# Rafae1130/qwen_inference_engine

Measured on AMD Instinct MI355X. Metric: decode tokens/s + prefill tok/s, Qwen2-7B bf16 batch=1, 1/2/4/8 MI355X, higher is better.
Workload: dtype bf16; 1 GPU; Qwen2-7B bf16 decode, batch=1, prompt=2048, gen=512; batch_per_gpu=1, batch=1, prompt=2048, gen=512, parallelism=single, graph=True, kv=contiguous

## Files before the change

### include/qie/qie_ops.h

```cpp
#ifndef QIE_OPS_H
#define QIE_OPS_H

#include "qie_types.h"

#ifdef __cplusplus
extern "C" {
#endif

#define QIE_ABI_VERSION 1

const char* qie_last_error(void);
int qie_abi_version(void);
int qie_device_count(int* count);

int qie_set_device(int device);
int qie_malloc(void** ptr, int64_t bytes);
int qie_free(void* ptr);
int qie_memcpy_h2d(void* dst, const void* src, int64_t bytes);
int qie_memcpy_d2h(void* dst, const void* src, int64_t bytes);
int qie_memset(void* ptr, int value, int64_t bytes);
int qie_synchronize(void);
int qie_stream_create(void** stream_out);
int qie_stream_synchronize(void* stream);
int qie_stream_destroy(void* stream);
// ... 23 lines not shown
    int64_t M, K, N;
    void* y;
    int64_t ldy;
    int32_t epilogue;
    int32_t numerics;
    const void* norm_w;
    float norm_eps;
    int32_t flags;
    uint64_t* argmax_keys;
    int64_t key_col0;
    const uint8_t* x_exps;
} qie_linear_args;

int qie_linear(const qie_linear_args* args, void* stream);

typedef struct qie_kv_cache {
    void* k;
    void* v;
    int64_t seq_stride;
    int32_t n_layers, n_kv_heads, head_dim, max_ctx;
    const int32_t* block_table;
    int32_t page_tokens;
    int32_t max_pages;
} qie_kv_cache;

int qie_qkv_post(const void* qkv, int64_t M, const int32_t* pos, int32_t rows_per_seq,
                 const void* q_norm, const void* k_norm, const float* rope_cos,
                 const float* rope_sin, int32_t n_heads, const qie_kv_cache* cache,
                 int32_t layer, float eps, int32_t numerics, void* q_out, void* stream);

int64_t qie_attention_workspace_bytes(int64_t M, int32_t n_heads, int32_t head_dim,
                                      int32_t max_ctx);
int qie_attention(const void* q, int64_t M, const int32_t* pos, int32_t rows_per_seq,
                  const qie_kv_cache* cache, int32_t layer, int32_t n_heads, void* out,
                  void* ws, void* stream);

int64_t qie_attention_extend_workspace_bytes(int64_t M, int32_t n_heads, int32_t head_dim,
                                             int32_t max_ctx);
int32_t qie_attention_extend_split_tokens(int64_t M, int32_t max_ctx);
int qie_attention_extend(const void* q, int64_t M, const int32_t* pos, int32_t rows_per_seq,
                         const qie_kv_cache* cache, int32_t layer, int32_t n_heads, void* out,
                         void* ws, void* stream);

#define QIE_NUMERICS_MASK 0xff
#define QIE_ATTN_PREROPED 0x100
int64_t qie_attention_decode_workspace_bytes(int64_t B, int32_t n_heads, int32_t n_kv_heads,
                                             int32_t head_dim, int32_t max_ctx);
int qie_attention_decode(const void* qkv, int64_t B, const int32_t* pos, const void* q_norm,
                         const void* k_norm, const float* rope_cos, const float* rope_sin,
                         int32_t n_heads, const qie_kv_cache* cache, int32_t layer, float eps,
                         int32_t numerics, void* out, void* ws, void* stream);

int qie_debug_tr16_probe(int32_t* out_dev);

int qie_qknorm(void* x, int64_t rows, int64_t row_stride, int32_t n_heads, int32_t head_dim,
               const void* w, float eps, int32_t numerics, void* stream);
int qie_rope(void* x, int64_t rows, int64_t row_stride, int32_t n_heads, int32_t head_dim,
             const int32_t* pos, int32_t pos0, const float* rope_cos, const float* rope_sin,
             int32_t numerics, void* stream);
int qie_kv_write(const void* k, const void* v, int64_t rows, int64_t ld, int32_t pos0,
                 const qie_kv_cache* cache, int32_t seq, int32_t layer, void* stream);

int qie_silu(void* x, int64_t n, void* stream);
int qie_mul(const void* a, const void* b, void* c, int64_t n, void* stream);
int qie_memcpy_d2d(void* dst, const void* src, int64_t bytes, void* stream);
int qie_silu_mul(const void* gate, const void* up, void* h, int64_t n, void* stream);
int qie_residual_add(void* x, const void* y, int64_t n, void* stream);
int qie_residual_add_f32(void* x, const float* sum, int64_t n, void* stream);

int64_t qie_sample_workspace_bytes(int64_t M, int64_t V);
int qie_sample(const void* logits, int64_t M, int64_t V, int64_t ld, const qie_sampling* s,
               const int32_t* step_dev, int32_t* out_ids, void* ws, void* stream);
int qie_keys_to_ids(const uint64_t* keys, int64_t M, int32_t* out_ids, void* stream);

uint32_t qie_tensor_id(const char* name);
int qie_synthetic_fill(void* dev, int64_t n, uint32_t tensor_id, uint64_t seed, float scale,
                       float offset, void* stream);
int qie_synthetic_fill_host(void* host, int64_t n, uint32_t tensor_id, uint64_t seed,
                            float scale, float offset);
#define QIE_LINEAR_FP8 1
#define QIE_LINEAR_TILE256 2
#define QIE_LINEAR_TILE128 4
#define QIE_LINEAR_STREAMK 8
int64_t qie_fp8_weight_bytes(int64_t rows, int64_t cols);
int qie_quantize_fp8(const void* w_bf16, int64_t rows, int64_t cols, void* out, void* stream);
int qie_quantize_fp8_host(const void* w_bf16, int64_t rows, int64_t cols, void* out);
int qie_dequantize_fp8(const void* w_fp8, int64_t rows, int64_t cols, void* out_bf16, void* stream);
#define QIE_LINEAR_FP8_T16 16
#define QIE_LINEAR_ACT_FP8 32
int qie_quantize_rows_fp8(const void* x, int64_t ldx, int64_t rows, int64_t cols, void* q, int64_t ldq,
                          void* exps, void* stream);
int qie_fp8_tile16(const void* w_fp8, int64_t rows, int64_t cols, void* out, void* stream);
int qie_debug_fp8_decode(float* out_dev);
int qie_debug_fp8_decode_bf16(uint16_t* out_dev);

int qie_synthetic_fill_slice(void* dev, int64_t rows, int64_t cols, int64_t full_cols, int64_t row0,
                             int64_t col0, uint32_t tensor_id, uint64_t seed, float scale, float offset,
                             void* stream);
int qie_scale_rows_pow2(void* w, int64_t rows, int64_t cols, int64_t row0, int64_t every, int32_t log2f,
                        void* stream);

#ifdef __cplusplus
}
#endif

#endif
```

### qwen_inference_engine_amd/_lib.py

```python
from __future__ import annotations

import ctypes as C
import os

_HERE = os.path.dirname(os.path.abspath(__file__))
LIB_PATH = os.environ.get("QIE_LIB") or os.path.join(_HERE, "lib", "libqie.so")

QIE_NUMERICS_REF = 0
QIE_NUMERICS_HF = 1
QIE_EPI_STORE = 0
QIE_EPI_RESIDUAL = 1
QIE_EPI_SWIGLU = 2
QIE_EPI_F32 = 3
QIE_LINEAR_FP8 = 1
QIE_LINEAR_TILE256 = 2
QIE_LINEAR_TILE128 = 4
QIE_LINEAR_STREAMK = 8
QIE_LINEAR_FP8_T16 = 16
QIE_LINEAR_ACT_FP8 = 32
QIE_ATTN_PREROPED = 0x100
QIE_COMM_ID_BYTES = 128
QIE_COMM_PEER_HANDLE_BYTES = 128


class ModelSpecC(C.Structure):
    _fields_ = [
        ("n_layers", C.c_int32), ("hidden", C.c_int32), ("n_heads", C.c_int32),
        ("n_kv_heads", C.c_int32), ("head_dim", C.c_int32), ("ffn", C.c_int32),
        ("vocab", C.c_int32), ("tie_embeddings", C.c_int32), ("qkv_bias", C.c_int32),
        ("qk_norm", C.c_int32), ("rms_eps", C.c_float), ("rope_theta", C.c_float),
        ("numerics", C.c_int32), ("reserved", C.c_int32 * 7),
    ]


class LayerWeightsC(C.Structure):
    _fields_ = [(n, C.c_void_p) for n in (
        "attn_norm", "wq", "wk", "wv", "bq", "bk", "bv", "q_norm", "k_norm", "wo",
        "ffn_norm", "w_gate", "w_up", "w_down")]


class ModelWeightsC(C.Structure):
    _fields_ = [("embed", C.c_void_p), ("final_norm", C.c_void_p), ("lm_head", C.c_void_p),
                ("n_layers", C.c_int32), ("layers", C.POINTER(LayerWeightsC))]


class SamplingC(C.Structure):
    _fields_ = [("top_k", C.c_int32), ("temperature", C.c_float), ("top_p", C.c_float),
                ("seed", C.c_uint64)]


class LinearArgsC(C.Structure):
    _fields_ = [
        ("x", C.c_void_p), ("ldx", C.c_int64), ("w", C.c_void_p * 3), ("bias", C.c_void_p * 3),
        ("seg_rows", C.c_int64 * 3), ("M", C.c_int64), ("K", C.c_int64), ("N", C.c_int64),
        ("y", C.c_void_p), ("ldy", C.c_int64), ("epilogue", C.c_int32), ("numerics", C.c_int32),
        ("norm_w", C.c_void_p), ("norm_eps", C.c_float), ("flags", C.c_int32),
        ("argmax_keys", C.c_void_p), ("key_col0", C.c_int64), ("x_exps", C.c_void_p),
    ]


class KvCacheC(C.Structure):
    _fields_ = [("k", C.c_void_p), ("v", C.c_void_p), ("seq_stride", C.c_int64),
                ("n_layers", C.c_int32), ("n_kv_heads", C.c_int32), ("head_dim", C.c_int32),
                ("max_ctx", C.c_int32), ("block_table", C.c_void_p), ("page_tokens", C.c_int32),
                ("max_pages", C.c_int32)]


class EngineOptsC(C.Structure):
    _fields_ = [("device", C.c_int32), ("max_ctx", C.c_int32), ("use_graph", C.c_int32),
                ("tp_rank", C.c_int32), ("tp_size", C.c_int32), ("tp_comm", C.c_void_p),
                ("weight_fp8", C.c_int32), ("comm_always", C.c_int32), ("prefill_fp8", C.c_int32),
                ("reserved", C.c_int32 * 5)]


_P = C.c_void_p
_I32, _I64, _U32, _U64, _F = C.c_int32, C.c_int64, C.c_uint32, C.c_uint64, C.c_float
_PI32 = C.POINTER(C.c_int32)
_PI64 = C.POINTER(C.c_int64)
_PF = C.POINTER(C.c_float)
_PD = C.POINTER(C.c_double)
_PCC = C.POINTER(C.c_char_p)
SIGNATURES = [
    ("qie_last_error", C.c_char_p, []),
    ("qie_abi_version", C.c_int, []),
    ("qie_device_count", C.c_int, [C.POINTER(C.c_int)]),
    ("qie_set_device", C.c_int, [C.c_int]),
    ("qie_malloc", C.c_int, [C.POINTER(_P), _I64]),
    ("qie_free", C.c_int, [_P]),
    ("qie_memcpy_h2d", C.c_int, [_P, _P, _I64]),
    ("qie_memcpy_d2h", C.c_int, [_P, _P, _I64]),
    ("qie_memset", C.c_int, [_P, C.c_int, _I64]),
    ("qie_synchronize", C.c_int, []),
    ("qie_stream_create", C.c_int, [C.POINTER(_P)]),
    ("qie_stream_synchronize", C.c_int, [_P]),
    ("qie_stream_destroy", C.c_int, [_P]),
    ("qie_rope_table_host", C.c_int, [_PF, _PF, _I32, _I32, _F, _I32]),
    ("qie_embedding", C.c_int, [_P, _P, _P, _I64, _I64, _P]),
    ("qie_rmsnorm", C.c_int, [_P, _P, _P, _I64, _I64, _F, _I32, _P]),
    ("qie_linear", C.c_int, [C.POINTER(LinearArgsC), _P]),
    ("qie_qkv_post", C.c_int, [_P, _I64, _P, _I32, _P, _P, _P, _P, _I32, C.POINTER(KvCacheC),
                               _I32, _F, _I32, _P, _P]),
    ("qie_attention_workspace_bytes", C.c_int64, [_I64, _I32, _I32, _I32]),
# ... 118 lines not shown
```

### qwen_inference_engine_amd/csrc/k_gemm.hip

```cpp
#include "qie_common.hpp"
#include "launch_util.hpp"
#include "../../include/qie/qie_ops.h"

#include <map>
#include <mutex>

namespace qie {

typedef __bf16 bf16x8 __attribute__((ext_vector_type(8)));
typedef float f32x4 __attribute__((ext_vector_type(4)));

struct GemmParams {
    const uint16_t* A;
    int64_t lda;
    const uint16_t* w0;
    const uint16_t* w1;
    const uint16_t* w2;
    const uint16_t* b0;
    const uint16_t* b1;
    const uint16_t* b2;
    int64_t n0, n01;
    int64_t M, K, N;
    int64_t wrows;
    uint16_t* C;
    int64_t ldc;
};

constexpr int BM = 128, BN = 128, BK = 64;

template <int EPI>
__device__ __forceinline__ const uint16_t* w_row(const GemmParams& p, int64_t nblk, int c, bool& valid, int eb,
                                                 int64_t& row, float& scale) {
    auto at = [&](const uint16_t* w, int64_t rows, int64_t r) {
        const uint8_t* b = reinterpret_cast<const uint8_t*>(w);
        scale = eb == 1 ? reinterpret_cast<const float*>(b + rows * p.K)[r] : 1.f;
        row = r;
        return reinterpret_cast<const uint16_t*>(b + r * p.K * eb);
    };
    if constexpr (EPI == QIE_EPI_SWIGLU) {
        const int64_t j = nblk * 64 + 32 * (c >> 6) + (c & 31);
        valid = j < p.N;
        const int64_t jj = valid ? j : p.N - 1;
        return ((c >> 5) & 1) ? at(p.w1, p.N, jj) : at(p.w0, p.N, jj);
    } else {
        const int64_t r = nblk * BN + c;
        valid = r < p.N;
        const int64_t rr = valid ? r : p.N - 1;
        if (rr < p.n0) return at(p.w0, p.n0, rr);
        if (rr < p.n01) return at(p.w1, p.n01 - p.n0, rr - p.n0);
        return at(p.w2, p.N - p.n01, rr - p.n01);
    }
}

__device__ __forceinline__ uint4 fp8x8_to_bf16(uint2 q, float sc) {
    float f[8];
    fp8x4_to_f32(q.x, f);
    fp8x4_to_f32(q.y, f + 4);
    return make_uint4(pack2(f[0] * sc, f[1] * sc), pack2(f[2] * sc, f[3] * sc), pack2(f[4] * sc, f[5] * sc),
                      pack2(f[6] * sc, f[7] * sc));
}

template <int EPI, int WT>
__global__ __launch_bounds__(256) void gemm_kernel(GemmParams p) {
#pragma clang fp contract(off)
    extern __shared__ __attribute__((aligned(16))) unsigned char smem[];
    uint16_t* As = reinterpret_cast<uint16_t*>(smem);
    uint16_t* Bs = reinterpret_cast<uint16_t*>(smem + 2 * BM * BK * 2);

    const int tid = threadIdx.x, lane = tid & 63, wave = tid >> 6;
    const int wr = wave >> 1, wc = wave & 1;
    const int64_t mblk = blockIdx.x, nblk = blockIdx.y;
    const int64_t m0 = mblk * BM;

    const uint16_t* a_src[4];
    const uint8_t* b_src[4];
    float b_sc[4];
    int lds_off[4];
    constexpr int EB = WT ? 1 : 2;
#pragma unroll
    for (int i = 0; i < 4; i++) {
        const int c = tid + 256 * i;
        const int row = c >> 3, ch = c & 7;
        int64_t ar = m0 + row;
        if (ar >= p.M) ar = p.M - 1;
// ... 225 lines not shown
        const uint16_t* Bs = As + TM * TK;
        bf16x8 af[8], bfr[NJ];
#pragma unroll
        for (int j = 0; j < NJ; j++) {
            const int row = wn * (BNT / 4) + j * 16 + fr;
            bfr[j] = *reinterpret_cast<const bf16x8*>(Bs + row * TK + ((g ^ big_swz(row)) * 8));
        }
#pragma unroll
        for (int i = 0; i < 8; i++) {
            const int row = wm * 128 + i * 16 + fr;
            af[i] = *reinterpret_cast<const bf16x8*>(As + row * TK + ((g ^ big_swz(row)) * 8));
        }
        __builtin_amdgcn_sched_barrier(0);
#pragma unroll
        for (int i = 0; i < 8; i++)
#pragma unroll
            for (int j = 0; j < NJ; j++)
                acc[i][j] = __builtin_amdgcn_mfma_f32_16x16x32_bf16(af[i], bfr[j], acc[i][j], 0, 0, 0);
    }

    if constexpr (EPI == QIE_EPI_SWIGLU) {
#pragma unroll
        for (int i = 0; i < 8; i++) {
#pragma unroll
            for (int jj = 0; jj < NJ / 2; jj++) {
                const int64_t col = nt * (BNT / 2) + (BNT / 8) * wn + 16 * jj + fr;
                if (col >= p.N) continue;
#pragma unroll
                for (int r = 0; r < 4; r++) {
                    const int64_t row = m0 + wm * 128 + i * 16 + g * 4 + r;
                    if (row >= p.M) continue;
                    const float gg = rbf(acc[i][jj][r]);
                    const float uu = rbf(acc[i][jj + NJ / 2][r]);
                    const float av = rbf(gg * (1.0f / (1.0f + expf(-gg))));
                    p.C[row * p.ldc + col] = f2bf(uu * av);
                }
            }
        }
    } else {
#pragma unroll
        for (int j = 0; j < NJ; j++) {
            const int64_t col = nt * BNT + wn * (BNT / 4) + j * 16 + fr;
            if (col >= p.N) continue;
            float bias = 0.f;
            if constexpr (EPI == QIE_EPI_STORE) {
                const uint16_t* b = col < p.n0 ? p.b0 : (col < p.n01 ? p.b1 : p.b2);
                if (b) bias = bf2f(b[col < p.n0 ? col : (col < p.n01 ? col - p.n0 : col - p.n01)]);
            }
#pragma unroll
            for (int i = 0; i < 8; i++) {
#pragma unroll
                for (int r = 0; r < 4; r++) {
                    const int64_t row = m0 + wm * 128 + i * 16 + g * 4 + r;
                    if (row >= p.M) continue;
                    if constexpr (EPI == QIE_EPI_F32) {
                        reinterpret_cast<float*>(p.C)[row * p.ldc + col] = acc[i][j][r];
                        continue;
                    }
                    uint16_t* dst = p.C + row * p.ldc + col;
                    if constexpr (EPI == QIE_EPI_RESIDUAL)
                        *dst = f2bf(bf2f(*dst) + rbf(acc[i][j][r]));
                    else
                        *dst = f2bf(acc[i][j][r] + bias);
                }
            }
        }
    }
}

typedef unsigned int u32x4_g8 __attribute__((ext_vector_type(4)));
namespace g8 {
constexpr int BM = 256, BN = 256, BK = 64;
constexpr int BUF = (BM + BN) * BK * 2;
}

__device__ __forceinline__ int g8_swz(int r) { return (r >> 1) & 7; }

struct G8Split {
    int splitk;
    float* slab;
    unsigned* cnt;
};

template <int EPI>
__global__ __launch_bounds__(512) void gemm8_kernel(GemmParams p, int n_mt, G8Split sk) {
#pragma clang fp contract(off)
    extern __shared__ __attribute__((aligned(16))) unsigned char smem[];
    const int tid = threadIdx.x, lane = tid & 63;
    const int wave = __builtin_amdgcn_readfirstlane(tid >> 6);
    const int wm = wave >> 2, wn = wave & 3;
    const int fr = lane & 15, g = lane >> 4;
    const int nwg = gridDim.x, orig = blockIdx.x;
    const int q8 = nwg >> 3, r8 = nwg & 7, xcd = orig & 7;
    const int wid = (xcd < r8 ? xcd * (q8 + 1) : r8 * (q8 + 1) + (xcd - r8) * q8) + (orig >> 3);
    const int tile = wid / sk.splitk, part = wid % sk.splitk;
    const int64_t mt = tile % n_mt, nt = tile / n_mt;
    const int64_t m0 = mt * g8::BM;

    const uint16_t* src[4][2];
    int dst_row[4][2];
#pragma unroll
    for (int u = 0; u < 4; u++)
#pragma unroll
        for (int i = 0; i < 2; i++) {
            const int b = 2 * wave + i;
            int row0;
            if (u == 0 || u == 3) row0 = (b < 8 ? 8 * b : 128 + 8 * (b - 8)) + (u == 3 ? 64 : 0);
            else row0 = 64 * (b >> 2) + 8 * (b & 3) + (u == 2 ? 32 : 0);
            dst_row[u][i] = row0;
            const int r = row0 + (lane >> 3);
            const int cs = (lane & 7) ^ g8_swz(r);
            if (u == 0 || u == 3) {
                int64_t ar = m0 + r;
                ar = ar < p.M ? ar : p.M - 1;
                src[u][i] = p.A + ar * p.lda + cs * 8;
            } else {
                src[u][i] = big_wrow<EPI, 256>(p, nt, r) + cs * 8;
            }
        }
    const int nk_all = (int)(p.K / g8::BK);
    const int kb = (int)((int64_t)part * nk_all / sk.splitk);
    const int nk = (int)((int64_t)(part + 1) * nk_all / sk.splitk) - kb;
    auto stage = [&](int u, int kt) {
        unsigned char* buf = smem + (kt & 1) * g8::BUF + ((u == 0 || u == 3) ? 0 : g8::BM * 128);
        const int64_t k0 = (int64_t)(kb + kt) * g8::BK;
#pragma unroll
        for (int i = 0; i < 2; i++) glds16(src[u][i] + k0, buf + dst_row[u][i] * 128);
    };

    f32x4 acc[8][4];
#pragma unroll
    for (int i = 0; i < 8; i++)
#pragma unroll
        for (int j = 0; j < 4; j++) acc[i][j] = f32x4{0.f, 0.f, 0.f, 0.f};
    bf16x8 fa[4][2], fb0[2][2], fb1[2][2];

    auto read_a = [&](const unsigned char* buf, int qa) {
#pragma unroll
        for (int i = 0; i < 4; i++)
#pragma unroll
            for (int s2 = 0; s2 < 2; s2++) {
                const int row = 128 * wm + 64 * qa + 16 * i + fr;
                fa[i][s2] = *reinterpret_cast<const bf16x8*>(buf + row * 128 + (((4 * s2 + g) ^ g8_swz(row)) * 16));
            }
    };
    auto read_b = [&](const unsigned char* buf, int qb, bf16x8 (&fb)[2][2]) {
#pragma unroll
        for (int j = 0; j < 2; j++)
#pragma unroll
            for (int s2 = 0; s2 < 2; s2++) {
                const int row = 64 * wn + 32 * qb + 16 * j + fr;
                fb[j][s2] = *reinterpret_cast<const bf16x8*>(buf + g8::BM * 128 + row * 128 +
                                                             (((4 * s2 + g) ^ g8_swz(row)) * 16));
            }
    };
    auto mfma_q = [&](int qa, int qb, const bf16x8 (&fb)[2][2]) {
        asm volatile("s_waitcnt lgkmcnt(0)" ::: "memory");
        __builtin_amdgcn_sched_barrier(0);
        __builtin_amdgcn_s_setprio(1);
#pragma unroll
        for (int s2 = 0; s2 < 2; s2++)
#pragma unroll
            for (int i = 0; i < 4; i++)
#pragma unroll
                for (int j = 0; j < 2; j++)
                    acc[4 * qa + i][2 * qb + j] =
                        __builtin_amdgcn_mfma_f32_16x16x32_bf16(fa[i][s2], fb[j][s2], acc[4 * qa + i][2 * qb + j], 0, 0, 0);
        __builtin_amdgcn_s_setprio(0);
        __builtin_amdgcn_sched_barrier(0);
    };
    auto bar = [&]() {
        __builtin_amdgcn_sched_barrier(0);
        __builtin_amdgcn_s_barrier();
        __builtin_amdgcn_sched_barrier(0);
    };
    auto wait8 = [&](bool tail) {
        if (tail) asm volatile("s_waitcnt vmcnt(0)" ::: "memory");
        else asm volatile("s_waitcnt vmcnt(8)" ::: "memory");
    };

    stage(0, 0); stage(1, 0); stage(2, 0); stage(3, 0);
    stage(0, 1); stage(1, 1);
    asm volatile("s_waitcnt vmcnt(8)" ::: "memory");
    bar();
    if (wm == 1) bar();
    for (int t = 0; t < nk; t++) {
        const unsigned char* buf = smem + (t & 1) * g8::BUF;
        const bool tail = t >= nk - 2;
        read_b(buf, 0, fb0);
        __builtin_amdgcn_sched_barrier(0);
        read_a(buf, 0);
        __builtin_amdgcn_sched_barrier(0);
        if (t + 1 < nk) stage(2, t + 1);
        wait8(tail);
        bar();
        mfma_q(0, 0, fb0);
        bar();
        read_b(buf, 1, fb1);
        __builtin_amdgcn_sched_barrier(0);
        if (t + 1 < nk) stage(3, t + 1);
        wait8(tail);
        bar();
        mfma_q(0, 1, fb1);
        bar();
        read_a(buf, 1);
        __builtin_amdgcn_sched_barrier(0);
        if (t + 2 < nk) stage(0, t + 2);
        bar();
        mfma_q(1, 1, fb1);
        bar();
        if (t + 2 < nk) stage(1, t + 2);
        wait8(tail);
        bar();
        mfma_q(1, 0, fb0);
        bar();
    }
    if (wm == 0) bar();

    if (sk.splitk > 1) {
        const int64_t tb = (int64_t)tile * sk.splitk;
        const auto rs = __builtin_amdgcn_make_buffer_rsrc(sk.slab + (tb + part) * 65536, (short)0, 65536 * 4, 0x00020000);
#pragma unroll
        for (int i = 0; i < 8; i++)
#pragma unroll
            for (int j = 0; j < 4; j++)
                __builtin_amdgcn_raw_buffer_store_b128(__builtin_bit_cast(u32x4_g8, acc[i][j]), rs,
                                                       ((wave * 32 + i * 4 + j) * 64 + lane) * 16, 0, 16);
        asm volatile("s_waitcnt vmcnt(0)" ::: "memory");
        __syncthreads();
        int* flag = reinterpret_cast<int*>(smem);
        if (tid == 0) {
            const unsigned old = __hip_atomic_fetch_add(sk.cnt + tile, 1u, __ATOMIC_RELAXED, __HIP_MEMORY_SCOPE_AGENT);
            *flag = old == (unsigned)sk.splitk - 1 ? 1 : 0;
        }
        __syncthreads();
        if (*flag == 0) return;
#pragma unroll
        for (int i = 0; i < 8; i++)
#pragma unroll
            for (int j = 0; j < 4; j++) acc[i][j] = f32x4{0.f, 0.f, 0.f, 0.f};
        for (int q = 0; q < sk.splitk; q++) {
            const auto rq = __builtin_amdgcn_make_buffer_rsrc(sk.slab + (tb + q) * 65536, (short)0, 65536 * 4, 0x00020000);
#pragma unroll
            for (int i = 0; i < 8; i++)
#pragma unroll
                for (int j = 0; j < 4; j++) {
                    const f32x4 v = __builtin_bit_cast(f32x4, __builtin_amdgcn_raw_buffer_load_b128(
                                                                  rq, ((wave * 32 + i * 4 + j) * 64 + lane) * 16, 0, 16));
                    acc[i][j] = q == 0 ? v : acc[i][j] + v;
                }
        }
        if (tid == 0) __hip_atomic_store(sk.cnt + tile, 0u, __ATOMIC_RELAXED, __HIP_MEMORY_SCOPE_AGENT);
    }

    constexpr int NJ = 4;
    if constexpr (EPI == QIE_EPI_SWIGLU) {
#pragma unroll
        for (int i = 0; i < 8; i++) {
#pragma unroll
            for (int jj = 0; jj < NJ / 2; jj++) {
                const int64_t col = nt * 128 + 32 * wn + 16 * jj + fr;
                if (col >= p.N) continue;
#pragma unroll
                for (int r = 0; r < 4; r++) {
                    const int64_t row = m0 + wm * 128 + i * 16 + g * 4 + r;
                    if (row >= p.M) continue;
                    const float gg = rbf(acc[i][jj][r]);
                    const float uu = rbf(acc[i][jj + NJ / 2][r]);
                    const float av = rbf(gg * (1.0f / (1.0f + expf(-gg))));
                    p.C[row * p.ldc + col] = f2bf(uu * av);
                }
            }
        }
    } else {
#pragma unroll
        for (int j = 0; j < NJ; j++) {
            const int64_t col = nt * 256 + wn * 64 + j * 16 + fr;
            if (col >= p.N) continue;
            float bias = 0.f;
            if constexpr (EPI == QIE_EPI_STORE) {
                const uint16_t* b = col < p.n0 ? p.b0 : (col < p.n01 ? p.b1 : p.b2);
                if (b) bias = bf2f(b[col < p.n0 ? col : (col < p.n01 ? col - p.n0 : col - p.n01)]);
            }
#pragma unroll
            for (int i = 0; i < 8; i++) {
#pragma unroll
                for (int r = 0; r < 4; r++) {
                    const int64_t row = m0 + wm * 128 + i * 16 + g * 4 + r;
                    if (row >= p.M) continue;
                    if constexpr (EPI == QIE_EPI_F32) {
                        reinterpret_cast<float*>(p.C)[row * p.ldc + col] = acc[i][j][r];
                        continue;
                    }
                    uint16_t* dst = p.C + row * p.ldc + col;
                    if constexpr (EPI == QIE_EPI_RESIDUAL)
                        *dst = f2bf(bf2f(*dst) + rbf(acc[i][j][r]));
                    else
                        *dst = f2bf(acc[i][j][r] + bias);
                }
            }
        }
    }
}

struct G8Stream {
    int dp_rounds;
    int tiles;
    int chunk;
    float* slab;
    unsigned* cnt;
};

template <int EPI>
__global__ __launch_bounds__(512) void gemm8sk_kernel(GemmParams p, int n_mt, G8Stream sk) {
#pragma clang fp contract(off)
    extern __shared__ __attribute__((aligned(16))) unsigned char smem[];
    const int tid = threadIdx.x, lane = tid & 63;
    const int wave = __builtin_amdgcn_readfirstlane(tid >> 6);
    const int wm = wave >> 2, wn = wave & 3;
    const int fr = lane & 15, g = lane >> 4;
    const int nwg = gridDim.x, orig = blockIdx.x;
    const int q8 = nwg >> 3, r8 = nwg & 7, xcd = orig & 7;
    const int wid = (xcd < r8 ? xcd * (q8 + 1) : r8 * (q8 + 1) + (xcd - r8) * q8) + (orig >> 3);
    const int nk_all = (int)(p.K / g8::BK);

    int64_t m0 = 0, nt = 0;
    const uint16_t* src[4][2];
    int dst_row[4][2];
    auto set_tile = [&](int tile) {
        const int64_t mt = tile % n_mt;
        nt = tile / n_mt;
        m0 = mt * g8::BM;
#pragma unroll
        for (int u = 0; u < 4; u++)
#pragma unroll
            for (int i = 0; i < 2; i++) {
                const int b = 2 * wave + i;
                int row0;
                if (u == 0 || u == 3) row0 = (b < 8 ? 8 * b : 128 + 8 * (b - 8)) + (u == 3 ? 64 : 0);
                else row0 = 64 * (b >> 2) + 8 * (b & 3) + (u == 2 ? 32 : 0);
                dst_row[u][i] = row0;
                const int r = row0 + (lane >> 3);
                const int cs = (lane & 7) ^ g8_swz(r);
                if (u == 0 || u == 3) {
                    int64_t ar = m0 + r;
                    ar = ar < p.M ? ar : p.M - 1;
                    src[u][i] = p.A + ar * p.lda + cs * 8;
                } else {
                    src[u][i] = big_wrow<EPI, 256>(p, nt, r) + cs * 8;
                }
            }
    };
    int kb = 0;
    auto stage = [&](int u, int kt) {
        unsigned char* buf = smem + (kt & 1) * g8::BUF + ((u == 0 || u == 3) ? 0 : g8::BM * 128);
        const int64_t k0 = (int64_t)(kb + kt) * g8::BK;
#pragma unroll
        for (int i = 0; i < 2; i++) glds16(src[u][i] + k0, buf + dst_row[u][i] * 128);
    };

// ... 125 lines not shown
#pragma unroll
                for (int i = 0; i < 8; i++) {
#pragma unroll
                    for (int r = 0; r < 4; r++) {
                        const int64_t row = m0 + wm * 128 + i * 16 + g * 4 + r;
                        if (row >= p.M) continue;
                        if constexpr (EPI == QIE_EPI_F32) {
                            reinterpret_cast<float*>(p.C)[row * p.ldc + col] = acc[i][j][r];
                            continue;
                        }
                        uint16_t* dst = p.C + row * p.ldc + col;
                        if constexpr (EPI == QIE_EPI_RESIDUAL)
                            *dst = f2bf(bf2f(*dst) + rbf(acc[i][j][r]));
                        else
                            *dst = f2bf(acc[i][j][r] + bias);
                    }
                }
            }
        }
    };

    for (int r = 0; r < sk.dp_rounds; r++) {
        set_tile(r * nwg + wid);
        run(0, nk_all);
        epilogue();
        __syncthreads();
    }
    const int64_t base = (int64_t)sk.dp_rounds * nwg * nk_all;
    const int64_t total = (int64_t)sk.tiles * nk_all;
    const int64_t ustart = base + (int64_t)wid * sk.chunk;
    const int64_t uend = ustart + sk.chunk < total ? ustart + sk.chunk : total;
    for (int64_t u = ustart; u < uend;) {
        const int tile = (int)(u / nk_all);
        const int k0 = (int)(u % nk_all);
        const int k1 = (int)(uend - u < (int64_t)(nk_all - k0) ? k0 + (uend - u) : nk_all);
        set_tile(tile);
        run(k0, k1 - k0);
        bool emit = true;
        if (k0 != 0 || k1 != nk_all) {
            const int slot = u == ustart ? 0 : 1;
            const auto rs = __builtin_amdgcn_make_buffer_rsrc(sk.slab + ((int64_t)wid * 2 + slot) * 65536, (short)0,
                                                              65536 * 4, 0x00020000);
#pragma unroll
            for (int i = 0; i < 8; i++)
#pragma unroll
                for (int j = 0; j < 4; j++)
                    __builtin_amdgcn_raw_buffer_store_b128(__builtin_bit_cast(u32x4_g8, acc[i][j]), rs,
                                                           ((wave * 32 + i * 4 + j) * 64 + lane) * 16, 0, 16);
            asm volatile("s_waitcnt vmcnt(0)" ::: "memory");
            __syncthreads();
            const int64_t tu0 = (int64_t)tile * nk_all - base;
            const int wf = (int)(tu0 / sk.chunk), wl = (int)((tu0 + nk_all - 1) / sk.chunk);
            int* flag = reinterpret_cast<int*>(smem);
            if (tid == 0) {
                const unsigned old = __hip_atomic_fetch_add(sk.cnt + tile, 1u, __ATOMIC_RELAXED, __HIP_MEMORY_SCOPE_AGENT);
                *flag = old == (unsigned)(wl - wf) ? 1 : 0;
            }
            __syncthreads();
            emit = *flag != 0;
            if (emit) {
                for (int w2 = wf; w2 <= wl; w2++) {
                    const int64_t s2 = base + (int64_t)w2 * sk.chunk;
                    const int slot2 = s2 / nk_all == tile ? 0 : 1;
                    const auto rq = __builtin_amdgcn_make_buffer_rsrc(sk.slab + ((int64_t)w2 * 2 + slot2) * 65536,
                                                                      (short)0, 65536 * 4, 0x00020000);
#pragma unroll
                    for (int i = 0; i < 8; i++)
#pragma unroll
                        for (int j = 0; j < 4; j++) {
                            const f32x4 v = __builtin_bit_cast(f32x4, __builtin_amdgcn_raw_buffer_load_b128(
                                                                          rq, ((wave * 32 + i * 4 + j) * 64 + lane) * 16, 0, 16));
                            acc[i][j] = w2 == wf ? v : acc[i][j] + v;
                        }
                }
                if (tid == 0) __hip_atomic_store(sk.cnt + tile, 0u, __ATOMIC_RELAXED, __HIP_MEMORY_SCOPE_AGENT);
            }
        }
        if (emit) epilogue();
        u += k1 - k0;
        __syncthreads();
    }
}

template <int EPI>
static int launch_gemm8_t(const GemmParams& p, int n_mt, int n_tiles, const G8Split& sk, hipStream_t st) {
    const void* fn = (const void*)gemm8_kernel<EPI>;
    constexpr size_t shm = 2 * (size_t)g8::BUF;
    QIE_TRY(raise_dynamic_lds(fn, shm));
    hipLaunchKernelGGL((gemm8_kernel<EPI>), dim3((unsigned)(n_tiles * sk.splitk)), dim3(512), shm, st, p, n_mt, sk);
    QIE_LAUNCH_CHECK();
    return 0;
}
static int launch_gemm8(int epi, const GemmParams& p, int n_mt, int n_tiles, const G8Split& sk, hipStream_t st) {
    return dispatch_epi(epi, [&](auto E) { return launch_gemm8_t<decltype(E)::value>(p, n_mt, n_tiles, sk, st); });
}

struct G8Ws {
    float* slab = nullptr;
    unsigned* cnt = nullptr;
    size_t slab_bytes = 0, cnt_n = 0;
};
static std::mutex g8_mu;
static std::map<hipStream_t, G8Ws> g8_ws;

static int g8_workspace(hipStream_t st, int slabs, int tiles, G8Split* out) {
    std::lock_guard<std::mutex> lk(g8_mu);
    G8Ws& w = g8_ws[st];
    const size_t need = (size_t)slabs * 65536 * 4;
    if (need > w.slab_bytes || (size_t)tiles > w.cnt_n) {
        hipStreamCaptureStatus cs = hipStreamCaptureStatusNone;
        if (hipStreamIsCapturing(st, &cs) != hipSuccess || cs != hipStreamCaptureStatusNone) return 1;
        QIE_HIP(hipStreamSynchronize(st));
        const size_t sb = std::max(need, w.slab_bytes), cn = std::max((size_t)tiles, w.cnt_n);
        if (w.slab) hipFree(w.slab);
        if (w.cnt) hipFree(w.cnt);
        w = G8Ws{};
        QIE_HIP(hipMalloc((void**)&w.slab, sb));
        QIE_HIP(hipMalloc((void**)&w.cnt, cn * 4));
        QIE_HIP(hipMemsetAsync(w.cnt, 0, cn * 4, st));
        w.slab_bytes = sb;
        w.cnt_n = cn;
    }
    out->slab = w.slab;
    out->cnt = w.cnt;
    return 0;
}

template <int EPI>
static int launch_gemm8sk_t(const GemmParams& p, int n_mt, int grid, const G8Stream& sk, hipStream_t st) {
    const void* fn = (const void*)gemm8sk_kernel<EPI>;
    constexpr size_t shm = 2 * (size_t)g8::BUF;
    QIE_TRY(raise_dynamic_lds(fn, shm));
    hipLaunchKernelGGL((gemm8sk_kernel<EPI>), dim3((unsigned)grid), dim3(512), shm, st, p, n_mt, sk);
    QIE_LAUNCH_CHECK();
    return 0;
}

static int launch_gemm8sk(int epi, const GemmParams& p, int n_mt, int tiles, hipStream_t st, bool* launched) {
    *launched = false;
    const int gk = dev_env("QIE_GEMM8_SK_GRID", 0);
    const int grid = gk > 0 ? gk : (int)device_cu_count();
    const int nk = (int)(p.K / g8::BK);
    G8Stream sk;
    sk.tiles = tiles;
    sk.dp_rounds = tiles / grid;
    const int64_t rest = (int64_t)(tiles - sk.dp_rounds * grid) * nk;
    sk.chunk = (int)std::max<int64_t>(1, (rest + grid - 1) / grid);
    G8Split ws{1, nullptr, nullptr};
    if (rest > 0 && g8_workspace(st, 2 * grid, tiles, &ws) != 0) return 0;
    sk.slab = ws.slab;
    sk.cnt = ws.cnt;
    *launched = true;
    return dispatch_epi(epi, [&](auto E) { return launch_gemm8sk_t<decltype(E)::value>(p, n_mt, grid, sk, st); });
}

static int g8_splitk(int64_t tiles, int64_t cus, int nk) {
    int best = 1;
    double best_t = 1e30;
    const int mink = std::max(4, dev_env("QIE_GEMM8_SK_MINK", 64));
    for (int s = 1; s <= 4 && nk / s >= mink; s++) {
        const double t = (double)((tiles * s + cus - 1) / cus) / s;
        if (t < best_t - 1e-9) {
            best_t = t;
            best = s;
        }
    }
    return best;
}

template <int EPI, int BNT>
static int launch_gemm_big_t(const GemmParams& p, int n_mt, int n_tiles, hipStream_t st) {
    const void* fn = (const void*)gemm_big_kernel<EPI, BNT>;
    constexpr size_t shm = (size_t)big::SLOTS * big::slot_bytes(BNT);
    QIE_TRY(raise_dynamic_lds(fn, shm));
    hipLaunchKernelGGL((gemm_big_kernel<EPI, BNT>), dim3((unsigned)n_tiles), dim3(512), shm, st, p, n_mt);
    QIE_LAUNCH_CHECK();
    return 0;
}

template <int BNT>
static int launch_gemm_big(int epi, const GemmParams& p, int n_mt, int n_tiles, hipStream_t st) {
    return dispatch_epi(epi, [&](auto E) { return launch_gemm_big_t<decltype(E)::value, BNT>(p, n_mt, n_tiles, st); });
}

template <int WT>
static int launch_gemm(int epi, unsigned gm, const GemmParams& p, size_t shm, hipStream_t st) {
    return dispatch_epi(epi, [&](auto E) {
        constexpr int EPI = decltype(E)::value;
        const unsigned gn = (unsigned)cdiv(p.N, EPI == QIE_EPI_SWIGLU ? 64 : BN);
        hipLaunchKernelGGL((gemm_kernel<EPI, WT>), dim3(gm, gn), dim3(256), shm, st, p);
        QIE_LAUNCH_CHECK();
        return 0;
    });
}

namespace mx {
constexpr int BK = 128;
}

struct MxParams {
    const uint8_t* A;
    int64_t lda;
    const uint8_t* ea;
    const uint8_t* w[3];
    const uint16_t* b[3];
    int64_t rows[3];
    int64_t n0, n01;
    int64_t M, K, N;
    uint16_t* C;
    int64_t ldc;
};

template <int EPI>
__device__ __forceinline__ int mx_wrow(const MxParams& p, int64_t nt, int c, int64_t& r) {
    if constexpr (EPI == QIE_EPI_SWIGLU) {
        const int ws = c / 64, q = c % 64;
        const int64_t j = nt * 128 + ws * 32 + (q % 32);
        r = j < p.N ? j : p.N - 1;
        return q >= 32 ? 1 : 0;
    } else {
        int64_t rr = nt * 256 + c;
        rr = rr < p.N ? rr : p.N - 1;
        if (rr < p.n0) { r = rr; return 0; }
        if (rr < p.n01) { r = rr - p.n0; return 1; }
        r = rr - p.n01;
        return 2;
    }
}

typedef int i32x8_mx __attribute__((ext_vector_type(8)));

template <int EPI, bool T16>
__global__ __launch_bounds__(512) void gemm8mx_kernel(MxParams p, int n_mt, G8Split sk, int dbg) {
#pragma clang fp contract(off)
    extern __shared__ __attribute__((aligned(16))) unsigned char smem[];
    const int tid = threadIdx.x, lane = tid & 63;
    const int wave = __builtin_amdgcn_readfirstlane(tid >> 6);
    const int wm = wave >> 2, wn = wave & 3;
    const int fr = lane & 15, g = lane >> 4;
    const int nwg = gridDim.x, orig = blockIdx.x;
    const int q8 = nwg >> 3, r8 = nwg & 7, xcd = orig & 7;
    const int wid = (xcd < r8 ? xcd * (q8 + 1) : r8 * (q8 + 1) + (xcd - r8) * q8) + (orig >> 3);
    const int tile = wid / sk.splitk, part = wid % sk.splitk;
    const int64_t mt = tile % n_mt, nt = tile / n_mt;
    const int64_t m0 = mt * g8::BM;
    const int64_t K = p.K;

    uint32_t sa_pk[2] = {0u, 0u}, sb_pk = 0u;
#pragma unroll
    for (int q = 0; q < 8; q++) {
        int64_t ar = m0 + 128 * wm + 16 * q + fr;
// ... 257 lines not shown
    QIE_REQUIRE(a->norm_w == nullptr && a->argmax_keys == nullptr, "qie_linear: ACT_FP8 takes no fused norm / arg-max");
    QIE_REQUIRE(((int64_t)cdiv(a->M, 256) * 256) * a->ldx < ((int64_t)1 << 32),
                "qie_linear: ACT_FP8 with M (%lld) x ldx (%lld) >= 2^32 bytes of codes (split the rows)",
                (long long)a->M, (long long)a->ldx);
    if (t16)
        QIE_REQUIRE(a->epilogue == QIE_EPI_SWIGLU ? a->N % 16 == 0
                                                  : a->seg_rows[0] % 16 == 0 && a->seg_rows[1] % 16 == 0 &&
                                                        a->seg_rows[2] % 16 == 0,
                    "qie_linear: tiled fp8 segments must be whole 16-row tiles");
    MxParams p;
    p.A = (const uint8_t*)a->x;
    p.lda = a->ldx;
    p.ea = a->x_exps;
    for (int i = 0; i < 3; i++) {
        p.w[i] = (const uint8_t*)a->w[i];
        p.b[i] = (const uint16_t*)a->bias[i];
    }
    const bool sw = a->epilogue == QIE_EPI_SWIGLU;
    p.rows[0] = sw ? a->N : a->seg_rows[0];
    p.rows[1] = sw ? a->N : a->seg_rows[1];
    p.rows[2] = sw ? 0 : a->seg_rows[2];
    p.n0 = a->seg_rows[0];
    p.n01 = a->seg_rows[0] + a->seg_rows[1];
    p.M = a->M;
    p.K = a->K;
    p.N = a->N;
    p.C = (uint16_t*)a->y;
    p.ldc = a->ldy;
    const int64_t cols = sw ? 2 * a->N : a->N;
    const int64_t n_mt = cdiv(a->M, g8::BM), tiles = n_mt * cdiv(cols, 256);
    const int64_t cus = device_cu_count();
    const int nk = (int)(a->K / mx::BK);
    G8Split sk{1, nullptr, nullptr};
    if (2 * tiles <= cus) {
        int best = 1;
        double best_t = 1e30;
        const int smax = dev_env("QIE_MX_SPLITK_MAX", 4);
        for (int s = 1; s <= smax && nk / s >= 8; s++) {
            const double t = (double)((tiles * s + cus - 1) / cus) / s;
            if (t < best_t - 1e-9) {
                best_t = t;
                best = s;
            }
        }
        if (best > 1 && g8_workspace(st, (int)tiles * best, (int)tiles, &sk) == 0) sk.splitk = best;
    }
    return t16 ? launch_gemm8mx<true>(a->epilogue, p, (int)n_mt, (int)tiles, sk, st)
               : launch_gemm8mx<false>(a->epilogue, p, (int)n_mt, (int)tiles, sk, st);
}

int gemm(const qie_linear_args* a, hipStream_t st) {
    if (a->flags & QIE_LINEAR_ACT_FP8) return gemm_mx(a, st);
    QIE_REQUIRE(a->norm_w == nullptr, "qie_linear: fused RMSNorm is GEMV-only (M <= 8)");
    QIE_REQUIRE(a->argmax_keys == nullptr, "qie_linear: fused arg-max is GEMV-only (M <= 8)");
    GemmParams p;
    p.A = (const uint16_t*)a->x;
    p.lda = a->ldx;
    p.w0 = (const uint16_t*)a->w[0];
    p.w1 = (const uint16_t*)a->w[1];
    p.w2 = (const uint16_t*)a->w[2];
    p.b0 = (const uint16_t*)a->bias[0];
    p.b1 = (const uint16_t*)a->bias[1];
    p.b2 = (const uint16_t*)a->bias[2];
    p.n0 = a->seg_rows[0];
    p.n01 = a->seg_rows[0] + a->seg_rows[1];
    p.M = a->M;
    p.K = a->K;
    p.N = a->N;
    p.wrows = 0;
    p.C = (uint16_t*)a->y;
    p.ldc = a->ldy;
    const size_t shm = (size_t)2 * (BM + BN) * BK * 2;
    const unsigned gm = (unsigned)cdiv(a->M, BM);
    QIE_REQUIRE(a->K % 8 == 0, "qie_linear: GEMM needs K %% 8 == 0");
    if (!(a->flags & QIE_LINEAR_FP8) && a->K % big::BK == 0 && a->ldx % 8 == 0) {
        const int64_t cols = a->epilogue == QIE_EPI_SWIGLU ? 2 * a->N : a->N;
        const int64_t n_mt = cdiv(a->M, big::BM);
        const int64_t t256 = n_mt * cdiv(cols, 256), t128 = n_mt * cdiv(cols, 128);
        const int64_t cus = device_cu_count();
        const int force = (a->flags & QIE_LINEAR_TILE256) ? 1 : (a->flags & QIE_LINEAR_TILE128) ? 2
                                                                                            : dev_env("QIE_GEMM_BIG", -1);
        const bool g8ok = a->K % g8::BK == 0 && a->K >= 4 * g8::BK;
        const int g8mode = dev_env("QIE_GEMM8", 2);
        if (g8ok && ((a->flags & QIE_LINEAR_STREAMK) || (g8mode == 3 && force < 0 && a->M >= big::BM))) {
            bool launched = false;
            const int rc = launch_gemm8sk(a->epilogue, p, (int)n_mt, (int)t256, st, &launched);
            if (rc || launched) return rc;
        }
        if (g8ok && g8mode != 0 && force != 2 && (force == 1 || (force < 0 && a->M >= big::BM && t256 >= cus))) {
            G8Split sk{1, nullptr, nullptr};
            return launch_gemm8(a->epilogue, p, (int)n_mt, (int)t256, sk, st);
        }
        if (g8ok && g8mode == 2 && force < 0 && a->M >= big::BM && t256 < cus) {
            const int s = g8_splitk(t256, cus, (int)(a->K / g8::BK));
            G8Split sk{1, nullptr, nullptr};
            if ((s == 1 && 2 * t256 >= cus) || (s > 1 && g8_workspace(st, (int)t256 * s, (int)t256, &sk) == 0 && (sk.splitk = s) > 1))
                return launch_gemm8(a->epilogue, p, (int)n_mt, (int)t256, sk, st);
        }
        if (force == 1 || (force < 0 && a->M >= big::BM && t256 >= cus))
            return launch_gemm_big<256>(a->epilogue, p, (int)n_mt, (int)t256, st);
        if (force == 2 || (force < 0 && a->M >= big::BM && t128 >= (3 * cus) / 4 && t128 <= cus))
            return launch_gemm_big<128>(a->epilogue, p, (int)n_mt, (int)t128, st);
        if (force < 0 && a->M >= big::BM && t256 >= cus / 2 && t256 <= cus && t128 > cus)
            return launch_gemm_big<256>(a->epilogue, p, (int)n_mt, (int)t256, st);
    }
    if (a->flags & QIE_LINEAR_FP8) return launch_gemm<1>(a->epilogue, gm, p, shm, st);
    return launch_gemm<0>(a->epilogue, gm, p, shm, st);
}

}
```

Baseline: 367.6 tokens/s.

## Add 192- and 128-column gemm8 tile widths with a planner for undersubscribed GEMMs

Templates the gemm8 MFMA kernel on its column tile width (256, 192, 128), changing the LDS staging layout, per-wave fragment counts and vmcnt waits. A new tile planner picks a narrower width when 256-wide tiles would leave CUs idle, falling back to split-K or the existing paths otherwise. The aim is better CU occupancy for prefill GEMMs whose output column count gives fewer 256-wide tiles than CUs. Narrow tiles only support STORE/RESIDUAL epilogues and give up some operand reuse per tile.

Result: no change. 367.0 tokens/s (-0.2%).

```diff
diff --git a/include/qie/qie_ops.h b/include/qie/qie_ops.h
--- a/include/qie/qie_ops.h
+++ b/include/qie/qie_ops.h
@@ -129,6 +129,8 @@
 #define QIE_LINEAR_TILE256 2
 #define QIE_LINEAR_TILE128 4
 #define QIE_LINEAR_STREAMK 8
+#define QIE_LINEAR_TILE192 64
+#define QIE_LINEAR_G8_TILE128 128
 int64_t qie_fp8_weight_bytes(int64_t rows, int64_t cols);
 int qie_quantize_fp8(const void* w_bf16, int64_t rows, int64_t cols, void* out, void* stream);
 int qie_quantize_fp8_host(const void* w_bf16, int64_t rows, int64_t cols, void* out);
diff --git a/qwen_inference_engine_amd/_lib.py b/qwen_inference_engine_amd/_lib.py
--- a/qwen_inference_engine_amd/_lib.py
+++ b/qwen_inference_engine_amd/_lib.py
@@ -18,6 +18,8 @@
 QIE_LINEAR_STREAMK = 8
 QIE_LINEAR_FP8_T16 = 16
 QIE_LINEAR_ACT_FP8 = 32
+QIE_LINEAR_TILE192 = 64
+QIE_LINEAR_G8_TILE128 = 128
 QIE_ATTN_PREROPED = 0x100
 QIE_COMM_ID_BYTES = 128
 QIE_COMM_PEER_HANDLE_BYTES = 128
diff --git a/qwen_inference_engine_amd/csrc/gemm_tile_plan.hpp b/qwen_inference_engine_amd/csrc/gemm_tile_plan.hpp
--- /dev/null
+++ b/qwen_inference_engine_amd/csrc/gemm_tile_plan.hpp
@@ -0,0 +1,67 @@
+#pragma once
+
+#include <cstdint>
+
+namespace qie {
+
+constexpr int kG8BM = 256, kG8BK = 64;
+
+inline int gemm8_splitk(int64_t tiles, int64_t cus, int nk, int mink = 64) {
+    int best = 1;
+    double best_t = 1e30;
+    if (mink < 4) mink = 4;
+    for (int s = 1; s <= 4 && nk / s >= mink; s++) {
+        const double t = (double)((tiles * s + cus - 1) / cus) / s;
+        if (t < best_t - 1e-9) {
+            best_t = t;
+            best = s;
+        }
+    }
+    return best;
+}
+
+inline int64_t gemm8_tiles(int64_t M, int64_t cols, int bn) {
+    return ((M + kG8BM - 1) / kG8BM) * ((cols + bn - 1) / bn);
+}
+
+constexpr int kG8W256 = 1, kG8W192 = 2, kG8W128 = 4;
+constexpr int kG8WidthsAll = kG8W256 | kG8W192 | kG8W128;
+constexpr int kG8WidthsShipped = kG8W256 | kG8W192;
+constexpr int g8_width_bit(int bn) { return bn == 256 ? kG8W256 : bn == 192 ? kG8W192 : bn == 128 ? kG8W128 : 0; }
+inline int gemm8_tile_width(int64_t M, int64_t cols, int64_t cus, int widths = kG8WidthsAll, int enabled = kG8WidthsAll) {
+    if (M < kG8BM || cols <= 0 || cus <= 0) return 0;
+    if (gemm8_tiles(M, cols, 256) >= cus) return 256;
+    int best = 0;
+    for (const int bn : {256, 192, 128}) {
+        if (!(widths & g8_width_bit(bn))) continue;
+        const int64_t t = gemm8_tiles(M, cols, bn);
+        if (t > cus || 2 * t < cus) continue;
+        if (best == 0 || bn < best) best = bn;
+    }
+    if (best && !(enabled & g8_width_bit(best)))
+        return widths == kG8W256 ? 0 : gemm8_tile_width(M, cols, cus, kG8W256, enabled);
+    return best;
+}
+
+struct Gemm8Plan {
+    int bn = 0;
+    int splitk = 1;
+};
+inline Gemm8Plan gemm8_plan(int64_t M, int64_t cols, int64_t K, int64_t cus, int widths = kG8WidthsAll,
+                            int enabled = kG8WidthsAll, int mink = 64) {
+    Gemm8Plan pl;
+    if (K % kG8BK != 0 || K < 4 * kG8BK || M < kG8BM) return pl;
+    const int64_t t256 = gemm8_tiles(M, cols, 256);
+    if (t256 < cus) {
+        const int s = gemm8_splitk(t256, cus, (int)(K / kG8BK), mink);
+        if (s > 1) {
+            pl.bn = 256;
+            pl.splitk = s;
+            return pl;
+        }
+    }
+    pl.bn = gemm8_tile_width(M, cols, cus, widths, enabled);
+    return pl;
+}
+
+}
diff --git a/qwen_inference_engine_amd/csrc/k_gemm.hip b/qwen_inference_engine_amd/csrc/k_gemm.hip
--- a/qwen_inference_engine_amd/csrc/k_gemm.hip
+++ b/qwen_inference_engine_amd/csrc/k_gemm.hip
@@ -1,5 +1,6 @@
 #include "qie_common.hpp"
 #include "launch_util.hpp"
+#include "gemm_tile_plan.hpp"
 #include "../../include/qie/qie_ops.h"
 
 #include <map>
@@ -391,9 +392,16 @@
     unsigned* cnt;
 };
 
-template <int EPI>
+template <int EPI, int BN = 256>
 __global__ __launch_bounds__(512) void gemm8_kernel(GemmParams p, int n_mt, G8Split sk) {
 #pragma clang fp contract(off)
+    static_assert(BN == 256 || BN == 192 || BN == 128, "gemm8: column tile of 256, 192 or 128");
+    static_assert(EPI != QIE_EPI_SWIGLU || BN == 256, "gemm8: the SwiGLU column interleave is 256 wide");
+    constexpr int SW = BN / 4;
+    constexpr int NJ = BN / 64;
+    constexpr int NJ0 = (NJ + 1) / 2, NJ1 = NJ - NJ0;
+    constexpr int BUF = (g8::BM + BN) * g8::BK * 2;
+    auto ucnt = [](int u) { return u == 1 ? NJ0 : (u == 2 ? NJ1 : 2); };
     extern __shared__ __attribute__((aligned(16))) unsigned char smem[];
     const int tid = threadIdx.x, lane = tid & 63;
     const int wave = __builtin_amdgcn_readfirstlane(tid >> 6);
@@ -412,10 +420,12 @@
     for (int u = 0; u < 4; u++)
 #pragma unroll
         for (int i = 0; i < 2; i++) {
-            const int b = 2 * wave + i;
+            if (i >= ucnt(u)) continue;
+            const int b = ucnt(u) * wave + i;
             int row0;
             if (u == 0 || u == 3) row0 = (b < 8 ? 8 * b : 128 + 8 * (b - 8)) + (u == 3 ? 64 : 0);
-            else row0 = 64 * (b >> 2) + 8 * (b & 3) + (u == 2 ? 32 : 0);
+            else if (u == 1) row0 = SW * (b / (2 * NJ0)) + 8 * (b % (2 * NJ0));
+            else row0 = SW * (b / (2 * NJ1)) + 16 * NJ0 + 8 * (b % (2 * NJ1));
             dst_row[u][i] = row0;
             const int r = row0 + (lane >> 3);
             const int cs = (lane & 7) ^ g8_swz(r);
@@ -424,25 +434,26 @@
                 ar = ar < p.M ? ar : p.M - 1;
                 src[u][i] = p.A + ar * p.lda + cs * 8;
             } else {
-                src[u][i] = big_wrow<EPI, 256>(p, nt, r) + cs * 8;
+                src[u][i] = big_wrow<EPI, BN>(p, nt, r) + cs * 8;
             }
         }
     const int nk_all = (int)(p.K / g8::BK);
     const int kb = (int)((int64_t)part * nk_all / sk.splitk);
     const int nk = (int)((int64_t)(part + 1) * nk_all / sk.splitk) - kb;
     auto stage = [&](int u, int kt) {
-        unsigned char* buf = smem + (kt & 1) * g8::BUF + ((u == 0 || u == 3) ? 0 : g8::BM * 128);
+        unsigned char* buf = smem + (kt & 1) * BUF + ((u == 0 || u == 3) ? 0 : g8::BM * 128);
         const int64_t k0 = (int64_t)(kb + kt) * g8::BK;
 #pragma unroll
-        for (int i = 0; i < 2; i++) glds16(src[u][i] + k0, buf + dst_row[u][i] * 128);
-    };
-
-    f32x4 acc[8][4];
+        for (int i = 0; i < 2; i++)
+            if (i < ucnt(u)) glds16(src[u][i] + k0, buf + dst_row[u][i] * 128);
+    };
+
+    f32x4 acc[8][NJ];
 #pragma unroll
     for (int i = 0; i < 8; i++)
 #pragma unroll
-        for (int j = 0; j < 4; j++) acc[i][j] = f32x4{0.f, 0.f, 0.f, 0.f};
-    bf16x8 fa[4][2], fb0[2][2], fb1[2][2];
+        for (int j = 0; j < NJ; j++) acc[i][j] = f32x4{0.f, 0.f, 0.f, 0.f};
+    bf16x8 fa[4][2], fb0[NJ0][2], fb1[NJ1][2];
 
     auto read_a = [&](const unsigned char* buf, int qa) {
 #pragma unroll
@@ -453,17 +464,19 @@
                 fa[i][s2] = *reinterpret_cast<const bf16x8*>(buf + row * 128 + (((4 * s2 + g) ^ g8_swz(row)) * 16));
             }
     };
-    auto read_b = [&](const unsigned char* buf, int qb, bf16x8 (&fb)[2][2]) {
-#pragma unroll
-        for (int j = 0; j < 2; j++)
+    auto read_b = [&](const unsigned char* buf, int qb, auto& fb) {
+        constexpr int nj = (int)(sizeof(fb) / sizeof(fb[0]));
+#pragma unroll
+        for (int j = 0; j < nj; j++)
 #pragma unroll
             for (int s2 = 0; s2 < 2; s2++) {
-                const int row = 64 * wn + 32 * qb + 16 * j + fr;
+                const int row = SW * wn + 16 * NJ0 * qb + 16 * j + fr;
                 fb[j][s2] = *reinterpret_cast<const bf16x8*>(buf + g8::BM * 128 + row * 128 +
                                                              (((4 * s2 + g) ^ g8_swz(row)) * 16));
             }
     };
-    auto mfma_q = [&](int qa, int qb, const bf16x8 (&fb)[2][2]) {
+    auto mfma_q = [&](int qa, int qb, const auto& fb) {
+        constexpr int nj = (int)(sizeof(fb) / sizeof(fb[0]));
         asm volatile("s_waitcnt lgkmcnt(0)" ::: "memory");
         __builtin_amdgcn_sched_barrier(0);
         __builtin_amdgcn_s_setprio(1);
@@ -472,9 +485,9 @@
 #pragma unroll
             for (int i = 0; i < 4; i++)
 #pragma unroll
-                for (int j = 0; j < 2; j++)
-                    acc[4 * qa + i][2 * qb + j] =
-                        __builtin_amdgcn_mfma_f32_16x16x32_bf16(fa[i][s2], fb[j][s2], acc[4 * qa + i][2 * qb + j], 0, 0, 0);
+                for (int j = 0; j < nj; j++)
+                    acc[4 * qa + i][NJ0 * qb + j] =
+                        __builtin_amdgcn_mfma_f32_16x16x32_bf16(fa[i][s2], fb[j][s2], acc[4 * qa + i][NJ0 * qb + j], 0, 0, 0);
         __builtin_amdgcn_s_setprio(0);
         __builtin_amdgcn_sched_barrier(0);
     };
@@ -482,19 +495,24 @@
         __builtin_amdgcn_sched_barrier(0);
         __builtin_amdgcn_s_barrier();
         __builtin_amdgcn_sched_barrier(0);
+    };
+    auto wait_units = [&]() {
+        if constexpr (NJ == 4) asm volatile("s_waitcnt vmcnt(8)" ::: "memory");
+        else if constexpr (NJ == 3) asm volatile("s_waitcnt vmcnt(7)" ::: "memory");
+        else asm volatile("s_waitcnt vmcnt(6)" ::: "memory");
     };
     auto wait8 = [&](bool tail) {
         if (tail) asm volatile("s_waitcnt vmcnt(0)" ::: "memory");
-        else asm volatile("s_waitcnt vmcnt(8)" ::: "memory");
+        else wait_units();
     };
 
     stage(0, 0); stage(1, 0); stage(2, 0); stage(3, 0);
     stage(0, 1); stage(1, 1);
-    asm volatile("s_waitcnt vmcnt(8)" ::: "memory");
+    wait_units();
     bar();
     if (wm == 1) bar();
     for (int t = 0; t < nk; t++) {
-        const unsigned char* buf = smem + (t & 1) * g8::BUF;
+        const unsigned char* buf = smem + (t & 1) * BUF;
         const bool tail = t >= nk - 2;
         read_b(buf, 0, fb0);
         __builtin_amdgcn_sched_barrier(0);
@@ -532,7 +550,7 @@
 #pragma unroll
         for (int i = 0; i < 8; i++)
 #pragma unroll
-            for (int j = 0; j < 4; j++)
+            for (int j = 0; j < NJ; j++)
                 __builtin_amdgcn_raw_buffer_store_b128(__builtin_bit_cast(u32x4_g8, acc[i][j]), rs,
                                                        ((wave * 32 + i * 4 + j) * 64 + lane) * 16, 0, 16);
         asm volatile("s_waitcnt vmcnt(0)" ::: "memory");
@@ -547,13 +565,13 @@
 #pragma unroll
         for (int i = 0; i < 8; i++)
 #pragma unroll
-            for (int j = 0; j < 4; j++) acc[i][j] = f32x4{0.f, 0.f, 0.f, 0.f};
+            for (int j = 0; j < NJ; j++) acc[i][j] = f32x4{0.f, 0.f, 0.f, 0.f};
         for (int q = 0; q < sk.splitk; q++) {
             const auto rq = __builtin_amdgcn_make_buffer_rsrc(sk.slab + (tb + q) * 65536, (short)0, 65536 * 4, 0x00020000);
 #pragma unroll
             for (int i = 0; i < 8; i++)
 #pragma unroll
-                for (int j = 0; j < 4; j++) {
+                for (int j = 0; j < NJ; j++) {
                     const f32x4 v = __builtin_bit_cast(f32x4, __builtin_amdgcn_raw_buffer_load_b128(
                                                                   rq, ((wave * 32 + i * 4 + j) * 64 + lane) * 16, 0, 16));
                     acc[i][j] = q == 0 ? v : acc[i][j] + v;
@@ -562,7 +580,6 @@
         if (tid == 0) __hip_atomic_store(sk.cnt + tile, 0u, __ATOMIC_RELAXED, __HIP_MEMORY_SCOPE_AGENT);
     }
 
-    constexpr int NJ = 4;
     if constexpr (EPI == QIE_EPI_SWIGLU) {
 #pragma unroll
         for (int i = 0; i < 8; i++) {
@@ -584,7 +601,7 @@
     } else {
 #pragma unroll
         for (int j = 0; j < NJ; j++) {
-            const int64_t col = nt * 256 + wn * 64 + j * 16 + fr;
+            const int64_t col = nt * BN + wn * SW + j * 16 + fr;
             if (col >= p.N) continue;
             float bias = 0.f;
             if constexpr (EPI == QIE_EPI_STORE) {
@@ -876,17 +893,25 @@
     }
 }
 
-template <int EPI>
+template <int EPI, int BN = 256>
 static int launch_gemm8_t(const GemmParams& p, int n_mt, int n_tiles, const G8Split& sk, hipStream_t st) {
-    const void* fn = (const void*)gemm8_kernel<EPI>;
-    constexpr size_t shm = 2 * (size_t)g8::BUF;
+    const void* fn = (const void*)gemm8_kernel<EPI, BN>;
+    constexpr size_t shm = 2 * (size_t)(g8::BM + BN) * g8::BK * 2;
     QIE_TRY(raise_dynamic_lds(fn, shm));
-    hipLaunchKernelGGL((gemm8_kernel<EPI>), dim3((unsigned)(n_tiles * sk.splitk)), dim3(512), shm, st, p, n_mt, sk);
+    hipLaunchKernelGGL((gemm8_kernel<EPI, BN>), dim3((unsigned)(n_tiles * sk.splitk)), dim3(512), shm, st, p, n_mt, sk);
     QIE_LAUNCH_CHECK();
     return 0;
 }
 static int launch_gemm8(int epi, const GemmParams& p, int n_mt, int n_tiles, const G8Split& sk, hipStream_t st) {
     return dispatch_epi(epi, [&](auto E) { return launch_gemm8_t<decltype(E)::value>(p, n_mt, n_tiles, sk, st); });
+}
+static bool gemm8_narrow_epi(int epi) { return epi == QIE_EPI_STORE || epi == QIE_EPI_RESIDUAL; }
+template <int BN>
+static int launch_gemm8_narrow(int epi, const GemmParams& p, int n_mt, const G8Split& sk, hipStream_t st) {
+    QIE_REQUIRE(gemm8_narrow_epi(epi), "qie_linear: the %d-column gemm8 tile has STORE and RESIDUAL epilogues only", BN);
+    const int n_tiles = n_mt * (int)cdiv(p.N, BN);
+    return epi == QIE_EPI_STORE ? launch_gemm8_t<QIE_EPI_STORE, BN>(p, n_mt, n_tiles, sk, st)
+                                : launch_gemm8_t<QIE_EPI_RESIDUAL, BN>(p, n_mt, n_tiles, sk, st);
 }
 
 struct G8Ws {
@@ -948,19 +973,6 @@
     return dispatch_epi(epi, [&](auto E) { return launch_gemm8sk_t<decltype(E)::value>(p, n_mt, grid, sk, st); });
 }
 
-static int g8_splitk(int64_t tiles, int64_t cus, int nk) {
-    int best = 1;
-    double best_t = 1e30;
-    const int mink = std::max(4, dev_env("QIE_GEMM8_SK_MINK", 64));
-    for (int s = 1; s <= 4 && nk / s >= mink; s++) {
-        const double t = (double)((tiles * s + cus - 1) / cus) / s;
-        if (t < best_t - 1e-9) {
-            best_t = t;
-            best = s;
-        }
-    }
-    return best;
-}
 
 template <int EPI, int BNT>
 static int launch_gemm_big_t(const GemmParams& p, int n_mt, int n_tiles, hipStream_t st) {
@@ -1384,6 +1396,16 @@
                                                                                             : dev_env("QIE_GEMM_BIG", -1);
         const bool g8ok = a->K % g8::BK == 0 && a->K >= 4 * g8::BK;
         const int g8mode = dev_env("QIE_GEMM8", 2);
+        {
+            int fbn = (a->flags & QIE_LINEAR_TILE192) ? 192 : (a->flags & QIE_LINEAR_G8_TILE128) ? 128 : 0;
+            if (fbn)
+                QIE_REQUIRE(g8ok, "qie_linear: the gemm8 tiles need K %% 64 == 0 and K >= 256 (K = %lld)", (long long)a->K);
+            else if (force < 0 && g8ok && a->M >= big::BM && gemm8_narrow_epi(a->epilogue))
+                fbn = dev_env("QIE_GEMM8_BN", 0);
+            const G8Split sk{1, nullptr, nullptr};
+            if (fbn == 192) return launch_gemm8_narrow<192>(a->epilogue, p, (int)n_mt, sk, st);
+            if (fbn == 128) return launch_gemm8_narrow<128>(a->epilogue, p, (int)n_mt, sk, st);
+        }
         if (g8ok && ((a->flags & QIE_LINEAR_STREAMK) || (g8mode == 3 && force < 0 && a->M >= big::BM))) {
             bool launched = false;
             const int rc = launch_gemm8sk(a->epilogue, p, (int)n_mt, (int)t256, st, &launched);
@@ -1394,10 +1416,22 @@
             return launch_gemm8(a->epilogue, p, (int)n_mt, (int)t256, sk, st);
         }
         if (g8ok && g8mode == 2 && force < 0 && a->M >= big::BM && t256 < cus) {
-            const int s = g8_splitk(t256, cus, (int)(a->K / g8::BK));
+            const int widths = gemm8_narrow_epi(a->epilogue) ? kG8WidthsAll : kG8W256;
+            const Gemm8Plan pl = gemm8_plan(a->M, cols, a->K, cus, widths, dev_env("QIE_GEMM8_WIDTHS", kG8WidthsShipped),
+                                            dev_env("QIE_GEMM8_SK_MINK", 64));
             G8Split sk{1, nullptr, nullptr};
-            if ((s == 1 && 2 * t256 >= cus) || (s > 1 && g8_workspace(st, (int)t256 * s, (int)t256, &sk) == 0 && (sk.splitk = s) > 1))
+            if (pl.splitk > 1) {
+                if (g8_workspace(st, (int)t256 * pl.splitk, (int)t256, &sk) == 0) {
+                    sk.splitk = pl.splitk;
+                    return launch_gemm8(a->epilogue, p, (int)n_mt, (int)t256, sk, st);
+                }
+            } else if (pl.bn == 256) {
                 return launch_gemm8(a->epilogue, p, (int)n_mt, (int)t256, sk, st);
+            } else if (pl.bn == 192) {
+                return launch_gemm8_narrow<192>(a->epilogue, p, (int)n_mt, sk, st);
+            } else if (pl.bn == 128) {
+                return launch_gemm8_narrow<128>(a->epilogue, p, (int)n_mt, sk, st);
+            }
         }
         if (force == 1 || (force < 0 && a->M >= big::BM && t256 >= cus))
             return launch_gemm_big<256>(a->epilogue, p, (int)n_mt, (int)t256, st);
```
